# maotian123/loc_lib

Hardware: AMD Instinct MI355X
Metric: scans/sec (64x1800-pt scan vs 10M-pt map) + ICP iter ms (higher is better)
Workload: dtype f64; 1 GPU; BASELINE configs[2]: 256 scans/GPU x 115200 pts (64x1800, cityblock-v1) vs one 10000000-pt map, P2PLANE ICP, reference defaults (alpha=0.1 KD-tree ANN, eps=1e-2, max 20 iters), scans sharded by rank, no collective; includes scan H2D: every step aligns a batch copied host->HBM for it (pinned double buffer, copy stream, overlapped with the previous step); 3 alignment(s) in flight; scans_per_gpu=256, map_points=10000000, pipeline_depth=3, search_mode=tree_faithful_ann, tree_depth=30, tree_bytes=239999992

## Files before the change

### loc_lib_amd/csrc/icp_kernels.hip

```cpp
#include "icp_kernels.hpp"
#include "launch.hpp"
#include "search_walk.hpp"
#include "../../include/locgpu.h"

#include <algorithm>
#include <cstdlib>

namespace locgpu {

template <int KMAX, int D, bool COUNT>
__global__ __launch_bounds__(kBlock) void icp_search_kernel(const uint2* __restrict__ tree, const float4* __restrict__ src,
                                                            const int* __restrict__ counts, const PoseState* __restrict__ st,
                                                            uint32_t* __restrict__ nn, size_t nn_pitch, int max_n, int k, float alpha_eff,
                                                            int skip_nonfinite, unsigned long long* __restrict__ visit_totals, uint32_t* __restrict__ touched,
                                                            const int* __restrict__ active, const int* __restrict__ src_of) {
    __shared__ uint32_t s_far[D][kBlock];
    __shared__ float s_d2[D][kBlock];
    const int scan = active ? active[blockIdx.y] : (int)blockIdx.y;
    if (st[scan].done) return;
    const int tid = threadIdx.x;
    const int i = blockIdx.x * kBlock + tid;
    if (i >= counts[scan]) return;
    const size_t gi = (size_t)scan * max_n + i;
    const float4 p = src[(size_t)(src_of ? src_of[scan] : scan) * max_n + i];
// ... 47 lines not shown
}

template <int K>
__device__ __forceinline__ bool walk_exact_in_wave(const uint2* __restrict__ tree, bool slow, float qx, float qy, float qz, float alpha_eff, uint2* lds,
                                                   uint32_t* __restrict__ nn, size_t nn_pitch, size_t gi, unsigned long long* __restrict__ search_stats) {
    const unsigned long long slow_mask = __ballot(slow);
    if (slow_mask == 0ull || __popcll(slow_mask) > 2) return slow_mask == 0ull;
    if (slow) {
        uint32_t(*s_far)[2] = reinterpret_cast<uint32_t(*)[2]>(lds);
        float(*s_d2)[2] = reinterpret_cast<float(*)[2]>(reinterpret_cast<char*>(lds) + 64 * 2 * sizeof(uint32_t));
        const int col = __popcll(slow_mask & ((1ull << (threadIdx.x & 63)) - 1ull));
        KnnHeap<K> heap;
        uint32_t nvis = 0, lvis = 0, out[K];
        int cnt;
        tree_knn_flat<K, 64, false, 2>(tree, qx, qy, qz, K, alpha_eff, s_far, s_d2, col, heap, nvis, lvis);
        heap_to_sorted<K>(heap, out, cnt);
#pragma unroll
        for (int j = 0; j < K; ++j) nn[(size_t)j * nn_pitch + gi] = out[j];
        if (search_stats) atomicAdd(&search_stats[1], 1ull);
    }
    return true;
}

template <int K, int DF, int LANES = 64, bool STAMP = false, int WIN = 0>
__global__ __launch_bounds__(64) void icp_search_walk_kernel(const uint2* __restrict__ tree, const float4* __restrict__ src,
                                                             const int* __restrict__ counts, const PoseState* __restrict__ st,
                                                             uint32_t* __restrict__ nn, size_t nn_pitch, int max_n, float alpha_eff, int T,
                                                             unsigned int tree_bytes, uint32_t dummy, int skip_nonfinite, uint32_t* __restrict__ redo_list,
                                                             unsigned int* __restrict__ redo_count, uint32_t* __restrict__ deep_list,
                                                             unsigned int* __restrict__ deep_count, unsigned long long* __restrict__ search_stats,
                                                             const int* __restrict__ active, const int* __restrict__ src_of) {
    extern __shared__ uint2 s_dyn[];
    constexpr int ROWB = LANES * 8;
    static_assert(DF * ROWB >= 64 * 2 * 8, "exact stack columns do not fit");
    if ((uint32_t)(size_t)s_dyn != 0u) __builtin_trap();
    const int scan = active ? active[blockIdx.y] : (int)blockIdx.y;
    const int tid = threadIdx.x;
    if (st[scan].done) return;
    const int i = blockIdx.x * LANES + tid;
    if (tid >= LANES || i >= counts[scan]) return;
    const size_t gi = (size_t)scan * max_n + i;
    const float4 p = load_once(&src[(size_t)(src_of ? src_of[scan] : scan) * max_n + i]);
    const bool finite = !skip_nonfinite || (isfinite(p.x) && isfinite(p.y) && isfinite(p.z));
    if (search_stats && finite) atomicAdd(&search_stats[0], 1ull);
    const D3 qs = se3_apply(st[scan].q, st[scan].t, D3{(double)p.x, (double)p.y, (double)p.z});
    const __amdgpu_buffer_rsrc_t rsrc = __builtin_amdgcn_make_buffer_rsrc((void*)tree, 0, (int)tree_bytes, 0x00020000);
    Walk<K> w;
    w.qx = (float)qs.x; w.qy = (float)qs.y; w.qz = (float)qs.z;
    static_assert(WIN <= DF - 2, "the window lies in the rows above the two candidate rows");
    walk_query<K, ROWB, STAMP, WIN>(rsrc, tree, w, finite, alpha_eff, T, dummy, (uint32_t)(size_t)(&s_dyn[tid]), DF);
    if (STAMP && search_stats) {
        atomicAdd(&search_stats[4], (unsigned long long)w.rounds);
        if ((tid & 63) == 0) { atomicAdd(&search_stats[9], (unsigned long long)w.wave_rounds); atomicAdd(&search_stats[12], 1ull); }
        atomicAdd(&search_stats[13], (unsigned long long)w.wave_rounds);
        redo_list[nn_pitch + gi] = w.rounds;
    }
    const bool deep = w.c3n == 1u;
    const bool slow = !deep && w.slow != 0u;
    if (!deep && !slow) {
#pragma unroll
        for (int j = 0; j < K; ++j) __builtin_nontemporal_store(w.id[j], &nn[(size_t)j * nn_pitch + gi]);
    }
    wave_append(deep_list, deep_count, deep, (uint32_t)gi);
    if (LANES == 16) {
        bool pending = slow;
        for (;;) {
            const unsigned long long m = __ballot(pending);
            if (m == 0ull) break;
            const bool mine = pending && __popcll(m & ((1ull << (threadIdx.x & 63)) - 1ull)) < 2;
            (void)walk_exact_in_wave<K>(tree, mine, w.qx, w.qy, w.qz, alpha_eff, s_dyn, nn, nn_pitch, gi, search_stats);
            pending = pending && !mine;
        }
    } else if (!walk_exact_in_wave<K>(tree, slow, w.qx, w.qy, w.qz, alpha_eff, s_dyn, nn, nn_pitch, gi, search_stats)) {
        wave_append(redo_list, redo_count, slow, (uint32_t)gi);
    }
}

template <int K, int D, int LANES = 64>
__global__ __launch_bounds__(64) void icp_search_walk_list_kernel(const uint2* __restrict__ tree, const float4* __restrict__ src,
                                                                  const PoseState* __restrict__ st, uint32_t* __restrict__ nn, size_t nn_pitch, int max_n,
                                                                  float alpha_eff, unsigned int tree_bytes, uint32_t dummy, const uint32_t* __restrict__ list,
                                                                  const unsigned int* __restrict__ n_list, uint32_t* __restrict__ redo_list,
                                                                  unsigned int* __restrict__ redo_count, unsigned long long* __restrict__ search_stats,
                                                                  const int* __restrict__ src_of) {
    extern __shared__ uint2 s_dyn[];
    constexpr int ROWB = LANES * 8;
    static_assert((D + 2) * ROWB >= 64 * 2 * 8, "exact stack columns do not fit");
    if ((uint32_t)(size_t)s_dyn != 0u) __builtin_trap();
    const unsigned int n = *n_list;
    const int tid = threadIdx.x;
    if (blockIdx.x == 0 && tid == 0 && search_stats) atomicAdd(&search_stats[2], (unsigned long long)n);
    if (tid >= LANES) return;
    const __amdgpu_buffer_rsrc_t rsrc = __builtin_amdgcn_make_buffer_rsrc((void*)tree, 0, (int)tree_bytes, 0x00020000);
    const unsigned int per_wave = min((unsigned int)LANES, max(1u, (n + gridDim.x - 1) / gridDim.x));
    for (unsigned int r0 = blockIdx.x * per_wave; r0 < n; r0 += gridDim.x * per_wave) {
        const unsigned int r = r0 + (unsigned int)tid;
        const bool valid = (unsigned int)tid < per_wave && r < n;
// ... 159 lines not shown
            double t = s_slice[0][threadIdx.x];
#pragma unroll
            for (int w = 1; w < kBlock / 32; ++w) t += s_slice[w][threadIdx.x];
            dst[threadIdx.x] = t;
        }
    }
};

__device__ __forceinline__ void R_hat(const double* R, const D3& q, double (&Rh)[3][3]) {
#pragma unroll
    for (int r = 0; r < 3; ++r) {
        Rh[r][0] = R[3 * r + 1] * q.z - R[3 * r + 2] * q.y;
        Rh[r][1] = R[3 * r + 2] * q.x - R[3 * r + 0] * q.z;
        Rh[r][2] = R[3 * r + 0] * q.y - R[3 * r + 1] * q.x;
    }
}


template <int FIT>
__global__ __launch_bounds__(kBlock) __attribute__((amdgpu_waves_per_eu(4, 4))) void icp_plane_accum_kernel(const uint2* __restrict__ tree, const float4* __restrict__ src,
                                                                 const int* __restrict__ counts, const PoseState* __restrict__ st,
                                                                 const uint32_t* __restrict__ nn, size_t nn_pitch, int max_n,
                                                                 double max_plane_distance, double* __restrict__ partials, int kPlanePts,
                                                                 const int* __restrict__ active, const int* __restrict__ src_of) {
    __shared__ double s_row[8][kAccPad];
    __shared__ double s_slice[kBlock / 32][32];
    const int scan = active ? active[blockIdx.y] : (int)blockIdx.y;
    if (st[scan].done) return;
    const int tid = threadIdx.x;
    RowAccum ra;
    ra.init();
#pragma unroll 1
    for (int pp = 0; pp < kPlanePts; ++pp) {
        const int i = (blockIdx.x * kPlanePts + pp) * kBlock + tid;
        double J[1][6] = {{0.0, 0.0, 0.0, 0.0, 0.0, 0.0}};
        double neg_e[1] = {0.0};
        double fitted = 0.0;
        if (i < counts[scan]) {
            const size_t gi = (size_t)scan * max_n + i;
            uint32_t slot[5];
#pragma unroll
            for (int j = 0; j < 5; ++j) slot[j] = __builtin_nontemporal_load(&nn[(size_t)j * nn_pitch + gi]);
            const float4 p = src[(size_t)(src_of ? src_of[scan] : scan) * max_n + i];
            if (slot[4] != kInvalidSlot) {
                D3 nb[5];
#pragma unroll
                for (int j = 0; j < 5; ++j) nb[j] = leaf_point(tree, slot[j]);
                double n4[4];
                if constexpr (FIT == 1) {
                    if (!plane_null_vector_secular(nb, n4)) plane_null_vector(nb, n4);
                } else {
                    plane_null_vector(nb, n4);
                }
                const D3 n3{n4[0], n4[1], n4[2]};
                bool fit = true;
#pragma unroll
                for (int j = 0; j < 5; ++j) {
// ... 1 lines not shown
                    if (err * err > 1e-2) fit = false;
                }
                if (fit) {
                    fitted = 1.0;
                    const D3 q{(double)p.x, (double)p.y, (double)p.z};
                    const D3 qs = se3_apply(st[scan].q, st[scan].t, q);
                    const double dis = dot3(n3, qs) + n4[3];
                    if (!(fabs(dis) > max_plane_distance)) {
                        const double* R = st[scan].R;
                        double nR[3];
#pragma unroll
                        for (int c = 0; c < 3; ++c) nR[c] = -n3.x * R[c] + (-n3.y * R[3 + c] + -n3.z * R[6 + c]);
                        J[0][0] = nR[1] * q.z - nR[2] * q.y;
                        J[0][1] = nR[2] * q.x - nR[0] * q.z;
                        J[0][2] = nR[0] * q.y - nR[1] * q.x;
                        J[0][3] = n3.x; J[0][4] = n3.y; J[0][5] = n3.z;
                        neg_e[0] = -dis;
                    }
                }
            }
        }
        ra.add<1>(s_row, J, neg_e, fitted);
    }
    ra.store(s_slice, partials + ((size_t)scan * gridDim.x + blockIdx.x) * kAccW);
}

__global__ __launch_bounds__(kBlock) void icp_point_accum_kernel(const uint2* __restrict__ tree, const float4* __restrict__ src,
                                                                 const int* __restrict__ counts, const PoseState* __restrict__ st,
                                                                 const uint32_t* __restrict__ nn, size_t nn_pitch, int max_n,
                                                                 double max_nn_distance, double* __restrict__ partials, int pts,
                                                                 const int* __restrict__ active, const int* __restrict__ src_of) {
    const int scan = active ? active[blockIdx.y] : (int)blockIdx.y;
    if (st[scan].done) return;
    double acc[28];
#pragma unroll
    for (int v = 0; v < 28; ++v) acc[v] = 0.0;
#pragma unroll 1
    for (int pp = 0; pp < pts; ++pp) {
    const int i = (blockIdx.x * pts + pp) * kBlock + threadIdx.x;
    if (i < counts[scan]) {
        const size_t gi = (size_t)scan * max_n + i;
        const uint32_t s0 = nn[gi];
        if (s0 != kInvalidSlot) {
            const float4 p = src[(size_t)(src_of ? src_of[scan] : scan) * max_n + i];
            const D3 q{(double)p.x, (double)p.y, (double)p.z};
            const D3 qs = se3_apply(st[scan].q, st[scan].t, q);
            const D3 e3 = leaf_point(tree, s0) - qs;
            const double dis2 = dot3(e3, e3);
            if (!(dis2 > max_nn_distance)) {
                acc[27] += 1.0;
                double Rh[3][3];
                R_hat(st[scan].R, q, Rh);
                double J[3][6];
#pragma unroll
                for (int r = 0; r < 3; ++r)
#pragma unroll
                    for (int c = 0; c < 3; ++c) { J[r][c] = Rh[r][c] / 16; J[r][3 + c] = (r == c) ? -1.0 : 0.0; }
                const double e[3] = {e3.x, e3.y, e3.z};
                add_rows<3>(acc, J, e);
            }
        }
    }
    }
    block_reduce_store<28>(acc, partials + ((size_t)scan * gridDim.x + blockIdx.x) * kAccW);
}

__global__ __launch_bounds__(kBlock) void icp_mapplane_accum_kernel(const double4* __restrict__ planes, const float4* __restrict__ src,
                                                                    const int* __restrict__ counts, const PoseState* __restrict__ st,
                                                                    const uint32_t* __restrict__ nn, int max_n, double max_plane_distance,
                                                                    double* __restrict__ partials, int pts, const int* __restrict__ active,
                                                                    const int* __restrict__ src_of) {
    const int scan = active ? active[blockIdx.y] : (int)blockIdx.y;
    if (st[scan].done) return;
    double acc[28];
#pragma unroll
    for (int v = 0; v < 28; ++v) acc[v] = 0.0;
    const int n = counts[scan];
    const size_t region = (size_t)(src_of ? src_of[scan] : scan) * max_n;
#pragma unroll 1
    for (int pp = 0; pp < pts; ++pp) {
        const int i = (blockIdx.x * pts + pp) * kBlock + threadIdx.x;
        if (i < n) {
            const uint32_t s0 = __builtin_nontemporal_load(&nn[(size_t)scan * max_n + i]);
            const float4 p = src[region + i];
            if (s0 != kInvalidSlot) {
                const double4 n4 = planes[s0 >> 1];
                if (n4.x == n4.x) {
                    acc[27] += 1.0;
                    const D3 n3{n4.x, n4.y, n4.z};
                    const D3 q{(double)p.x, (double)p.y, (double)p.z};
                    const D3 qs = se3_apply(st[scan].q, st[scan].t, q);
                    const double dis = dot3(n3, qs) + n4.w;
                    if (!(fabs(dis) > max_plane_distance)) {
                        const double* R = st[scan].R;
                        double nR[3];
#pragma unroll
                        for (int c = 0; c < 3; ++c) nR[c] = -n3.x * R[c] + (-n3.y * R[3 + c] + -n3.z * R[6 + c]);
                        double J[1][6];
                        J[0][0] = nR[1] * q.z - nR[2] * q.y;
                        J[0][1] = nR[2] * q.x - nR[0] * q.z;
                        J[0][2] = nR[0] * q.y - nR[1] * q.x;
                        J[0][3] = n3.x; J[0][4] = n3.y; J[0][5] = n3.z;
                        const double e[1] = {dis};
                        add_rows<1>(acc, J, e);
                    }
                }
            }
        }
    }
    block_reduce_store<28>(acc, partials + ((size_t)scan * gridDim.x + blockIdx.x) * kAccW);
}

__global__ __launch_bounds__(kBlock) __attribute__((amdgpu_waves_per_eu(5, 5))) void icp_line_accum_kernel(const uint2* __restrict__ tree, const float4* __restrict__ src,
                                                                const int* __restrict__ counts, const PoseState* __restrict__ st,
                                                                const uint32_t* __restrict__ nn, size_t nn_pitch, int max_n,
                                                                double max_line_distance, double* __restrict__ partials, int pts,
                                                                const int* __restrict__ active, const int* __restrict__ src_of) {
    __shared__ double s_row[8][kAccPad];
    __shared__ double s_slice[kBlock / 32][32];
    const int scan = active ? active[blockIdx.y] : (int)blockIdx.y;
    if (st[scan].done) return;
    RowAccum ra;
    ra.init();
#pragma unroll 1
    for (int pp = 0; pp < pts; ++pp) {
    const int i = (blockIdx.x * pts + pp) * kBlock + threadIdx.x;
    double J[3][6], neg_e[3] = {0.0, 0.0, 0.0};
    double fitted = 0.0;
#pragma unroll
    for (int r = 0; r < 3; ++r)
#pragma unroll
        for (int c = 0; c < 6; ++c) J[r][c] = 0.0;
    if (i < counts[scan]) {
        const size_t gi = (size_t)scan * max_n + i;
        uint32_t slot[5];
#pragma unroll
        for (int j = 0; j < 5; ++j) slot[j] = nn[(size_t)j * nn_pitch + gi];
        const float4 p = src[(size_t)(src_of ? src_of[scan] : scan) * max_n + i];
        if (slot[4] != kInvalidSlot) {
            const D3 q{(double)p.x, (double)p.y, (double)p.z};
            const D3 qs = se3_apply(st[scan].q, st[scan].t, q);
            D3 nb[5];
#pragma unroll
            for (int j = 0; j < 5; ++j) nb[j] = leaf_point(tree, slot[j]);
            D3 sum{0.0, 0.0, 0.0};
#pragma unroll
            for (int j = 0; j < 5; ++j) sum = sum + nb[j];
            const D3 p0{sum.x / 5.0, sum.y / 5.0, sum.z / 5.0};
            D3 dl[5];
// ... 23 lines not shown
                            s += hd[r][2] * R[6 + c];
                            hR[r][c] = s;
                        }
#pragma unroll
                    for (int r = 0; r < 3; ++r)
#pragma unroll
                        for (int c = 0; c < 3; ++c) {
                            double s = hR[r][0] * hq[0][c];
                            s += hR[r][1] * hq[1][c];
                            s += hR[r][2] * hq[2][c];
                            A[r][c] = s;
                        }
#pragma unroll
                    for (int r = 0; r < 3; ++r)
#pragma unroll
                        for (int c = 0; c < 3; ++c) { J[r][c] = -A[r][c]; J[r][3 + c] = hd[r][c]; }
                    neg_e[0] = -e3.x; neg_e[1] = -e3.y; neg_e[2] = -e3.z;
                }
            }
        }
    }
    ra.add<3>(s_row, J, neg_e, fitted);
    }
    ra.store(s_slice, partials + ((size_t)scan * gridDim.x + blockIdx.x) * kAccW);
}

__device__ __forceinline__ double reduce_partials(const double* __restrict__ rows, int blocks_per_scan, bool mine, double (*s_sum)[kAccW]) {
    const int col = threadIdx.x & (kAccW - 1), chunk = threadIdx.x / kAccW;
    constexpr int kChunks = kBlock / kAccW;
    double s = 0.0;
    if (mine && col < 28) {
        constexpr int kFlight = 32;
        for (int b = chunk; b < blocks_per_scan; b += kChunks * kFlight) {
            double v[kFlight];
#pragma unroll
            for (int u = 0; u < kFlight; ++u) {
                const int idx = b + u * kChunks;
                v[u] = idx < blocks_per_scan ? rows[(size_t)idx * kAccW + col] : 0.0;
            }
#pragma unroll
            for (int u = 0; u < kFlight; ++u) s += v[u];
        }
    }
    s_sum[chunk][col] = s;
    __syncthreads();
    double t = 0.0;
    if (threadIdx.x < kAccW) {
// ... 108 lines not shown
    if ((threadIdx.x & 63) == 0 && c) atomicAdd(&totals[3], c);
}

__global__ __launch_bounds__(kBlock) void transform_cloud_kernel(const float4* __restrict__ src, size_t n, M12f m, float* __restrict__ dst_xyz) {
    const size_t i = (size_t)blockIdx.x * kBlock + threadIdx.x;
    if (i >= n) return;
    const float4 p = src[i];
    const float* m12 = m.v;
    dst_xyz[3 * i + 0] = ((m12[0] * p.x + m12[1] * p.y) + m12[2] * p.z) + m12[3];
    dst_xyz[3 * i + 1] = ((m12[4] * p.x + m12[5] * p.y) + m12[6] * p.z) + m12[7];
    dst_xyz[3 * i + 2] = ((m12[8] * p.x + m12[9] * p.y) + m12[10] * p.z) + m12[11];
}

__global__ __launch_bounds__(kBlock) void nn_to_index_kernel(const uint2* __restrict__ tree, const uint32_t* __restrict__ nn, size_t nn_pitch, size_t n_queries,
                                                             int k, int32_t* __restrict__ out) {
    const size_t gi = (size_t)blockIdx.x * kBlock + threadIdx.x;
    if (gi >= n_queries) return;
    for (int j = 0; j < k; ++j) {
        const uint32_t slot = nn[(size_t)j * nn_pitch + gi];
        out[gi * k + j] = slot == kInvalidSlot ? -1 : (int32_t)(tree[slot].y & 0x3FFFFFFFu);
    }
}

void launch_nn_to_index(const uint2* tree, const uint32_t* nn, size_t nn_pitch, size_t n_queries, int k, int32_t* out, hipStream_t s) {
    hipLaunchKernelGGL(nn_to_index_kernel, dim3((unsigned)((n_queries + kBlock - 1) / kBlock)), dim3(kBlock), 0, s, tree, nn, nn_pitch, n_queries, k, out);
}

template <int KMAX, int D>
static void launch_search_kd(const SearchArgs& a, hipStream_t s) {
    dim3 grid((a.max_n + kBlock - 1) / kBlock, a.active ? a.n_active : a.n_scans);
    if (a.visit_totals)
        hipLaunchKernelGGL((icp_search_kernel<KMAX, D, true>), grid, dim3(kBlock), 0, s, a.tree, a.src, a.counts, a.st, a.nn, a.nn_pitch, a.max_n,
                           a.k, a.alpha_eff, a.skip_nonfinite, a.visit_totals, a.touched, a.active, a.src_of);
    else
        hipLaunchKernelGGL((icp_search_kernel<KMAX, D, false>), grid, dim3(kBlock), 0, s, a.tree, a.src, a.counts, a.st, a.nn, a.nn_pitch, a.max_n,
                           a.k, a.alpha_eff, a.skip_nonfinite, a.visit_totals, nullptr, a.active, a.src_of);
}

template <int KMAX>
static bool launch_search_k(const SearchArgs& a, hipStream_t s) {
    if (a.depth <= 32) launch_search_kd<KMAX, 32>(a, s);
    else if (a.depth <= 40) launch_search_kd<KMAX, 40>(a, s);
    else if (a.depth <= 64) launch_search_kd<KMAX, 64>(a, s);
    else return false;
    return true;
}
static int fast_stack_depth() {
    static int v = -1;
    if (v < 0) {
        const char* e = getenv("LOCGPU_FAST_STACK");
        v = e ? atoi(e) : 10;
        if (v != 12 && v != 15 && v != 24) v = 10;
    }
    return v;
}

template <auto Kernel>
static bool no_static_lds() {
    hipFuncAttributes attr{};
    return hipFuncGetAttributes(&attr, reinterpret_cast<const void*>(Kernel)) == hipSuccess && attr.sharedSizeBytes == 0;
}
template <int K, int D>
static bool walk_kernels_ok_kd() {
    return no_static_lds<icp_search_walk_kernel<K, 10, 64, false, 8>>() && no_static_lds<icp_search_walk_kernel<K, 12>>() && no_static_lds<icp_search_walk_kernel<K, 15>>() && no_static_lds<icp_search_walk_kernel<K, 24>>() &&
           no_static_lds<icp_search_walk_kernel<K, D + 2, 16>>() && no_static_lds<icp_search_walk_list_kernel<K, D, kDeepLanes>>();
}
bool search_kernels_lds_ok() {
    static const bool ok = walk_kernels_ok_kd<1, 32>() && walk_kernels_ok_kd<1, 40>() && walk_kernels_ok_kd<1, 64>() &&
                           walk_kernels_ok_kd<5, 32>() && walk_kernels_ok_kd<5, 40>() && walk_kernels_ok_kd<5, 64>();
    return ok;
}

template <int K, int D, int DF, int WIN = 0>
static bool launch_walk_kd(const SearchArgs& a, hipStream_t s) {
    static const bool stamp = [] { const char* e = getenv("LOCGPU_STAMP"); return e && atoi(e) != 0; }();
    const uint32_t dummy = (uint32_t)(a.tree_bytes / 8);
    const unsigned int rsrc_bytes = (unsigned int)a.tree_bytes + 16u;
    const int n_launch = a.active ? a.n_active : a.n_scans;
    if (!stamp && (size_t)((a.max_n + 63) / 64) * n_launch <= 2048) {
        dim3 g1((a.max_n + 15) / 16, n_launch);
        hipLaunchKernelGGL((icp_search_walk_kernel<K, D + 2, 16>), g1, dim3(64), (D + 2) * 16 * 8, s, a.tree, a.src, a.counts, a.st, a.nn, a.nn_pitch, a.max_n,
                           a.alpha_eff, 0, rsrc_bytes, dummy, a.skip_nonfinite, a.redo_list, a.redo_count, a.redo_list2, a.redo_count2, a.search_stats, a.active, a.src_of);
        return true;
    }
    static const int t_off = [] { const char* e = getenv("LOCGPU_K1_T_OFFSET"); const int v = e ? atoi(e) : 0; return v > 0 ? v : 13; }();
    const int stored = WIN ? t_off : DF - 2;
    const int Tw = a.depth > stored ? a.depth - stored : 0;
    dim3 g2((a.max_n + 63) / 64, n_launch);
    static const bool lds_knob = getenv("LOCGPU_K1_LDS_BYTES") != nullptr;
    unsigned lds_bytes = DF * 64 * 8;
    if (lds_knob) { const char* e = getenv("LOCGPU_K1_LDS_BYTES"); lds_bytes = (unsigned)std::max(e ? atoi(e) : 0, DF * 64 * 8); }
    if (stamp)
        hipLaunchKernelGGL((icp_search_walk_kernel<K, DF, 64, true, WIN>), g2, dim3(64), DF * 64 * 8, s, a.tree, a.src, a.counts, a.st, a.nn, a.nn_pitch, a.max_n,
                           a.alpha_eff, Tw, rsrc_bytes, dummy, a.skip_nonfinite, a.redo_list, a.redo_count, a.redo_list2, a.redo_count2, a.search_stats, a.active, a.src_of);
    else
        hipLaunchKernelGGL((icp_search_walk_kernel<K, DF, 64, false, WIN>), g2, dim3(64), lds_bytes, s, a.tree, a.src, a.counts, a.st, a.nn, a.nn_pitch, a.max_n,
                           a.alpha_eff, Tw, rsrc_bytes, dummy, a.skip_nonfinite, a.redo_list, a.redo_count, a.redo_list2, a.redo_count2, a.search_stats, a.active, a.src_of);
    hipLaunchKernelGGL((icp_search_walk_list_kernel<K, D, kDeepLanes>), dim3(kDeepWaves), dim3(64), (D + 2) * kDeepLanes * 8, s, a.tree, a.src, a.st, a.nn, a.nn_pitch, a.max_n,
                       a.alpha_eff, rsrc_bytes, dummy, a.redo_list2, a.redo_count2, a.redo_list, a.redo_count, a.search_stats, a.src_of);
    hipLaunchKernelGGL((icp_search_redo_kernel<K, D>), dim3(kRedoWaves), dim3(64), 0, s, a.tree, a.src, a.st, a.nn, a.nn_pitch, a.max_n, a.k,
                       a.alpha_eff, a.redo_list, a.redo_count, a.search_stats, a.src_of);
    return true;
}
template <int K, int D>
static bool launch_walk_d(const SearchArgs& a, hipStream_t s) {
    switch (fast_stack_depth()) {
        default: {
            static const int win = [] { const char* e = getenv("LOCGPU_K1_WIN"); return e ? atoi(e) : 8; }();
            if (win == 6) return launch_walk_kd<K, D, 10, 6>(a, s);
            if (win == 7) return launch_walk_kd<K, D, 10, 7>(a, s);
            return launch_walk_kd<K, D, 10, 8>(a, s);
        }
        case 12: {
            static const int win = [] { const char* e = getenv("LOCGPU_K1_WIN"); return e ? atoi(e) : 0; }();
            if (win == 8) return launch_walk_kd<K, D, 12, 8>(a, s);
            if (win == 9) return launch_walk_kd<K, D, 12, 9>(a, s);
            return launch_walk_kd<K, D, 12>(a, s);
        }
        case 24: return launch_walk_kd<K, D, 24>(a, s);
        case 15: return launch_walk_kd<K, D, 15>(a, s);
// ... 70 lines not shown
    if (depth <= 32) hipLaunchKernelGGL((knn_query_kernel<KMAX, 32>), grid, dim3(kBlock), 0, s, tree, q, nq, k, alpha_eff, out, visits);
    else if (depth <= 40) hipLaunchKernelGGL((knn_query_kernel<KMAX, 40>), grid, dim3(kBlock), 0, s, tree, q, nq, k, alpha_eff, out, visits);
    else if (depth <= 64) hipLaunchKernelGGL((knn_query_kernel<KMAX, 64>), grid, dim3(kBlock), 0, s, tree, q, nq, k, alpha_eff, out, visits);
    else return false;
    return true;
}
bool launch_knn_query(const uint2* tree, int depth, const float* q, size_t nq, int k, float alpha_eff, int32_t* out, uint32_t* visits,
                      hipStream_t s) {
    if (k == 1) return launch_knn_k<1>(tree, depth, q, nq, k, alpha_eff, out, visits, s);
    if (k <= 5) return launch_knn_k<5>(tree, depth, q, nq, k, alpha_eff, out, visits, s);
    if (k <= 8) return launch_knn_k<8>(tree, depth, q, nq, k, alpha_eff, out, visits, s);
    return false;
}

int icp_accum_split(int method, int max_n, int n_scans) {
    const long total_blocks = (long)((max_n + kBlock - 1) / kBlock) * n_scans;
    return total_blocks >= 8192 ? (method == 2 ? 4 : 8) : (total_blocks >= 4096 ? 4 : (total_blocks >= 2048 ? 2 : 1));
}

int launch_icp_accum(int method, const AccumArgs& a, hipStream_t s) {
    const int blocks = (a.max_n + kBlock - 1) / kBlock;
    int pts = icp_accum_split(method, a.max_n, a.n_scans);
    if (a.split_scans > 0) pts = icp_accum_split(method, a.max_n, a.split_scans);
    const dim3 grid((blocks + pts - 1) / pts, a.active ? a.n_active : a.n_scans);
    if (method == 2) {
        if (plane_fit_mode() == 1)
            hipLaunchKernelGGL(icp_plane_accum_kernel<1>, grid, dim3(kBlock), 0, s, a.tree, a.src, a.counts, a.st, a.nn, a.nn_pitch, a.max_n, a.gate, a.partials, pts, a.active, a.src_of);
        else
            hipLaunchKernelGGL(icp_plane_accum_kernel<0>, grid, dim3(kBlock), 0, s, a.tree, a.src, a.counts, a.st, a.nn, a.nn_pitch, a.max_n, a.gate, a.partials, pts, a.active, a.src_of);
    } else if (method == LOCGPU_P2PLANE_MAP)
        hipLaunchKernelGGL(icp_mapplane_accum_kernel, grid, dim3(kBlock), 0, s, reinterpret_cast<const double4*>(a.planes), a.src, a.counts, a.st, a.nn, a.max_n, a.gate, a.partials, pts, a.active, a.src_of);
    else if (method == 1)
        hipLaunchKernelGGL(icp_line_accum_kernel, grid, dim3(kBlock), 0, s, a.tree, a.src, a.counts, a.st, a.nn, a.nn_pitch, a.max_n, a.gate, a.partials, pts, a.active, a.src_of);
    else
        hipLaunchKernelGGL(icp_point_accum_kernel, grid, dim3(kBlock), 0, s, a.tree, a.src, a.counts, a.st, a.nn, a.nn_pitch, a.max_n, a.gate, a.partials, pts, a.active, a.src_of);
    return (int)grid.x;
}

void launch_gn_solve(const double* partials, int blocks_per_scan, PoseState* st, int n_scans, const GnParams& prm, int do_update, double* hb_out,
                     unsigned int* list_counts, hipStream_t s, const int* scans, const GnPost* post) {
    hipLaunchKernelGGL(gn_solve_kernel, dim3(n_scans), dim3(kBlock), 0, s, partials, blocks_per_scan, st, prm, do_update, hb_out, list_counts, scans, post ? *post : GnPost{});
}

void launch_sum_partials(const double* partials, int blocks_per_scan, const PoseState* st_all, int first, int n_local, int n_total, double* acc,
                         hipStream_t s, const unsigned char* owned) {
    hipLaunchKernelGGL(sum_partials_kernel, dim3(n_total), dim3(kBlock), 0, s, partials, blocks_per_scan, st_all, first, n_local, acc, owned);
}

void launch_count_touched(uint32_t* touched, size_t n_words, unsigned long long* totals, hipStream_t s) {
    hipLaunchKernelGGL(count_touched_kernel, dim3(1024), dim3(kBlock), 0, s, touched, n_words, totals);
}

void launch_transform_cloud(const float4* src, size_t n, const M12f& m12, float* dst_xyz, hipStream_t s) {
    hipLaunchKernelGGL(transform_cloud_kernel, dim3((unsigned)((n + kBlock - 1) / kBlock)), dim3(kBlock), 0, s, src, n, m12, dst_xyz);
}

}
```

### loc_lib_amd/csrc/icp_kernels.hpp

```cpp
#pragma once
#include <hip/hip_runtime.h>
#include <stdint.h>

#include "device_math.hpp"

namespace locgpu {

constexpr int kBlock = 256;
constexpr int kAccW = 32;
constexpr uint32_t kInvalidSlot = 0xFFFFFFFFu;
constexpr int kSearchStatSlots = 16 + 2 * 64;

struct GnParams {
    int method;
    int max_iteration;
    int min_effective_pts;
    double eps;
    double max_nn_distance, max_plane_distance, max_line_distance;
    bool operator==(const GnParams& o) const {
        return method == o.method && max_iteration == o.max_iteration && min_effective_pts == o.min_effective_pts && eps == o.eps &&
               max_nn_distance == o.max_nn_distance && max_plane_distance == o.max_plane_distance && max_line_distance == o.max_line_distance;
    }
};

__device__ __forceinline__ float as_f32(uint32_t u) { return __uint_as_float(u); }

__device__ __forceinline__ void wave_append(uint32_t* __restrict__ list, unsigned int* __restrict__ count, bool pred, uint32_t value) {
    const unsigned long long mask = __ballot(pred);
    if (!mask) return;
    const int lane = (int)__lane_id();
    const int leader = __ffsll((long long)mask) - 1;
    unsigned int base = 0;
    if (lane == leader) base = atomicAdd(count, (unsigned int)__popcll(mask));
    base = (unsigned int)__shfl((int)base, leader, 64);
    if (pred) list[base + (unsigned int)__popcll(mask & ((1ull << lane) - 1ull))] = value;
}

template <int KMAX>
struct KnnHeap {
    float d[KMAX + 1];
    uint32_t id[KMAX + 1];
    int n;

    __device__ __forceinline__ float getd(int i) const {
        float r = d[0];
// ... 213 lines not shown
```

### loc_lib_amd/csrc/launch.hpp

```cpp
#pragma once
#include "gn_post.hpp"
#include <hip/hip_runtime.h>
#include <stdint.h>

#include "device_math.hpp"

namespace locgpu {

struct GnParams;

struct SearchArgs {
    const uint2* tree;
    size_t tree_bytes;
    int depth;
    const float4* src;
    const int* counts;
    const PoseState* st;
    uint32_t* nn;
    size_t nn_pitch;
    int max_n, n_scans, k;
    float alpha_eff;
    int skip_nonfinite;
    unsigned long long* visit_totals;
    uint32_t* redo_list;
// ... 4 lines not shown
    const int* active = nullptr;
    int n_active = 0;
    const int* src_of = nullptr;
    uint32_t* touched = nullptr;
};

struct AccumArgs {
    const uint2* tree;
    const float4* src;
    const int* counts;
    const PoseState* st;
    const uint32_t* nn;
    size_t nn_pitch;
    int max_n, n_scans;
    double gate;
    double* partials;
    const int* active = nullptr;
    int n_active = 0;
    const int* src_of = nullptr;
    int split_scans = 0;
    const double* planes = nullptr;
};

bool launch_icp_search(const SearchArgs& a, hipStream_t s);
bool launch_icp_search_redo(const SearchArgs& a, hipStream_t s);
bool launch_icp_search_list(const SearchArgs& a, const uint32_t* list, const unsigned int* n_list, hipStream_t s);
bool launch_knn_query(const uint2* tree, int depth, const float* q, size_t nq, int k, float alpha_eff, int32_t* out, uint32_t* visits,
                      hipStream_t s);
int launch_icp_accum(int method, const AccumArgs& a, hipStream_t s);
void launch_gn_solve(const double* partials, int blocks_per_scan, PoseState* st, int n_scans, const GnParams& prm, int do_update, double* hb_out,
                     unsigned int* list_counts, hipStream_t s, const int* scans = nullptr, const GnPost* post = nullptr);
int icp_accum_split(int method, int max_n, int n_scans);
void launch_sum_partials(const double* partials, int blocks_per_scan, const PoseState* st_all, int first, int n_local, int n_total, double* acc,
                         hipStream_t s, const unsigned char* owned = nullptr);
constexpr int kFitW = 4;
struct FitnessArgs {
    const uint2* tree;
    const float4* src;
    const int* counts;
    const PoseState* st;
    const uint32_t* nn;
    int max_n, n_scans;
    float gate2;
    double* partials;
    double* out;
    unsigned int* list_counts;
// ... 17 lines not shown
```

### loc_lib_amd/csrc/locgpu_api.hip

```cpp
#include <algorithm>
#include <atomic>
#include <chrono>
#include <thread>
#include <cmath>
#include <cstdio>
#include <cstring>
#include <string>
#include <vector>

#include "batch_upload.hpp"
#include "context.hpp"
#include "cloud_filters.hpp"
#include "kdtree_build.hpp"
#include "launch.hpp"

#include <dlfcn.h>
#include <rccl/rccl.h>

using namespace locgpu;

namespace {
struct Rccl {
    ncclResult_t (*GetUniqueId)(ncclUniqueId*) = nullptr;
    ncclResult_t (*CommInitRank)(ncclComm_t*, int, ncclUniqueId, int) = nullptr;
// ... 155 lines not shown
int locgpu_create(int device_id, locgpu_ctx** out) {
    if (!out) return fail(nullptr, LOCGPU_ERR_INVALID, "locgpu_create: out is NULL");
    *out = nullptr;
    int n = 0;
    hipError_t e = hipGetDeviceCount(&n);
    if (e != hipSuccess || n <= 0)
        return fail(nullptr, LOCGPU_ERR_NO_DEVICE, std::string("no HIP device available (there is no CPU fallback): ") + hipGetErrorString(e));
    if (device_id < 0 || device_id >= n) return fail(nullptr, LOCGPU_ERR_INVALID, "locgpu_create: device_id out of range");
    auto* ctx = new locgpu_ctx();
    ctx->device = device_id;
    locgpu_ndt_opts_default(&ctx->ndt_opts);
    bool ok = hip_ok(nullptr, hipSetDevice(device_id), "hipSetDevice");
    for (int i = 0; ok && i < locgpu_ctx::kSlots; ++i) ok = hip_ok(nullptr, hipStreamCreateWithFlags(&ctx->slot_stream[i], hipStreamNonBlocking), "hipStreamCreate");
    ok = ok && hip_ok(nullptr, hipStreamCreateWithFlags(&ctx->copy_stream, hipStreamNonBlocking), "hipStreamCreate");
    ok = ok && hip_ok(nullptr, hipStreamCreateWithFlags(&ctx->comm_stream, hipStreamNonBlocking), "hipStreamCreate");
    if (!ok) {
        for (hipStream_t st : ctx->slot_stream) if (st) (void)hipStreamDestroy(st);
        if (ctx->copy_stream) (void)hipStreamDestroy(ctx->copy_stream);
        if (ctx->comm_stream) (void)hipStreamDestroy(ctx->comm_stream);
        delete ctx;
        return LOCGPU_ERR_NO_DEVICE;
    }
    ctx->stream = ctx->slot_stream[0];
    if (!search_kernels_lds_ok()) {
        locgpu_destroy(ctx);
        return fail(nullptr, LOCGPU_ERR_INVALID, "locgpu_create: a search kernel of this build owns static LDS — its traversal stack would not start at LDS address 0 (search_walk.hpp)");
    }
    *out = ctx;
    return LOCGPU_OK;
}

void locgpu_destroy(locgpu_ctx* ctx) {
    if (!ctx) return;
    (void)hipSetDevice(ctx->device);
    (void)target_join(ctx, false);
    free_target_scratch(ctx);
    for (hipStream_t st : ctx->slot_stream) if (st) (void)hipStreamSynchronize(st);
    if (ctx->comm_stream) (void)hipStreamSynchronize(ctx->comm_stream);
    delete ctx->worker;
    free_batch(ctx->single);
    free_batch(ctx->search);
    free_batch(ctx->planes_ws);
    if (ctx->d_planes) (void)hipFree(ctx->d_planes);
    if (ctx->d_planes_count) (void)hipFree(ctx->d_planes_count);
    upload_free_ctx(ctx);
    if (ctx->comm) { (void)rccl().CommDestroy((ncclComm_t)ctx->comm); ctx->comm = nullptr; }
// ... 1819 lines not shown
```

Before: 12140 scans/s.

## Flatten search walk and accumulate kernels into grid-stride loops over virtual tiles

The walk-search kernel and the ICP accumulate kernels now launch a flat 1-D grid. Each block loops over a virtual (scan, tile) index described by a new VGrid struct, instead of reading blockIdx.x/y directly. The grid size can be capped at a per-CU multiple of the device CU count, queried at context creation, or set through environment knobs. The per-CU constants are zero, so by default the grid still equals the total tile count. The walk kernel also gains an amdgpu_waves_per_eu(8) occupancy hint, which can change register allocation. The change lays groundwork for persistent, machine-sized grids, at the cost of an integer divide per tile and extra __syncthreads in the accumulate loops.

```diff
diff --git a/loc_lib_amd/csrc/icp_kernels.hip b/loc_lib_amd/csrc/icp_kernels.hip
--- a/loc_lib_amd/csrc/icp_kernels.hip
+++ b/loc_lib_amd/csrc/icp_kernels.hip
@@ -93,22 +93,17 @@
     return true;
 }
 
-template <int K, int DF, int LANES = 64, bool STAMP = false, int WIN = 0>
-__global__ __launch_bounds__(64) void icp_search_walk_kernel(const uint2* __restrict__ tree, const float4* __restrict__ src,
-                                                             const int* __restrict__ counts, const PoseState* __restrict__ st,
-                                                             uint32_t* __restrict__ nn, size_t nn_pitch, int max_n, float alpha_eff, int T,
-                                                             unsigned int tree_bytes, uint32_t dummy, int skip_nonfinite, uint32_t* __restrict__ redo_list,
-                                                             unsigned int* __restrict__ redo_count, uint32_t* __restrict__ deep_list,
-                                                             unsigned int* __restrict__ deep_count, unsigned long long* __restrict__ search_stats,
-                                                             const int* __restrict__ active, const int* __restrict__ src_of) {
-    extern __shared__ uint2 s_dyn[];
+template <int K, int DF, int LANES, bool STAMP, int WIN>
+__device__ __forceinline__ void walk_tile(uint2* s_dyn, int scan, int tile, const uint2* __restrict__ tree, const float4* __restrict__ src,
+                                          const int* __restrict__ counts, const PoseState* __restrict__ st, uint32_t* __restrict__ nn, size_t nn_pitch,
+                                          int max_n, float alpha_eff, int T, unsigned int tree_bytes, uint32_t dummy, int skip_nonfinite,
+                                          uint32_t* __restrict__ redo_list, unsigned int* __restrict__ redo_count, uint32_t* __restrict__ deep_list,
+                                          unsigned int* __restrict__ deep_count, unsigned long long* __restrict__ search_stats,
+                                          const int* __restrict__ src_of) {
     constexpr int ROWB = LANES * 8;
-    static_assert(DF * ROWB >= 64 * 2 * 8, "exact stack columns do not fit");
-    if ((uint32_t)(size_t)s_dyn != 0u) __builtin_trap();
-    const int scan = active ? active[blockIdx.y] : (int)blockIdx.y;
     const int tid = threadIdx.x;
     if (st[scan].done) return;
-    const int i = blockIdx.x * LANES + tid;
+    const int i = tile * LANES + tid;
     if (tid >= LANES || i >= counts[scan]) return;
     const size_t gi = (size_t)scan * max_n + i;
     const float4 p = load_once(&src[(size_t)(src_of ? src_of[scan] : scan) * max_n + i]);
@@ -144,6 +139,32 @@
         }
     } else if (!walk_exact_in_wave<K>(tree, slow, w.qx, w.qy, w.qz, alpha_eff, s_dyn, nn, nn_pitch, gi, search_stats)) {
         wave_append(redo_list, redo_count, slow, (uint32_t)gi);
+    }
+}
+
+template <int K, int DF, int LANES = 64, bool STAMP = false, int WIN = 0, bool LOOP = false>
+__global__ __launch_bounds__(64) __attribute__((amdgpu_waves_per_eu(8))) void icp_search_walk_kernel(const uint2* __restrict__ tree, const float4* __restrict__ src,
+                                                             const int* __restrict__ counts, const PoseState* __restrict__ st,
+                                                             uint32_t* __restrict__ nn, size_t nn_pitch, int max_n, float alpha_eff, int T,
+                                                             unsigned int tree_bytes, uint32_t dummy, int skip_nonfinite, uint32_t* __restrict__ redo_list,
+                                                             unsigned int* __restrict__ redo_count, uint32_t* __restrict__ deep_list,
+                                                             unsigned int* __restrict__ deep_count, unsigned long long* __restrict__ search_stats,
+                                                             const int* __restrict__ active, const int* __restrict__ src_of, VGrid vg) {
+    extern __shared__ uint2 s_dyn[];
+    static_assert(DF * LANES * 8 >= 64 * 2 * 8, "exact stack columns do not fit");
+    if ((uint32_t)(size_t)s_dyn != 0u) __builtin_trap();
+    if constexpr (LOOP) {
+#pragma unroll 1
+        for (int v = blockIdx.x; v < vg.total; v += gridDim.x) {
+            const int vy = v / vg.per_scan, vx = v - vy * vg.per_scan;
+            const int scan = active ? active[vy] : vy;
+            walk_tile<K, DF, LANES, STAMP, WIN>(s_dyn, scan, vx, tree, src, counts, st, nn, nn_pitch, max_n, alpha_eff, T, tree_bytes, dummy, skip_nonfinite,
+                                                redo_list, redo_count, deep_list, deep_count, search_stats, src_of);
+        }
+    } else {
+        const int scan = active ? active[blockIdx.y] : (int)blockIdx.y;
+        walk_tile<K, DF, LANES, STAMP, WIN>(s_dyn, scan, (int)blockIdx.x, tree, src, counts, st, nn, nn_pitch, max_n, alpha_eff, T, tree_bytes, dummy, skip_nonfinite,
+                                            redo_list, redo_count, deep_list, deep_count, search_stats, src_of);
     }
 }
 
@@ -349,17 +370,20 @@
                                                                  const int* __restrict__ counts, const PoseState* __restrict__ st,
                                                                  const uint32_t* __restrict__ nn, size_t nn_pitch, int max_n,
                                                                  double max_plane_distance, double* __restrict__ partials, int kPlanePts,
-                                                                 const int* __restrict__ active, const int* __restrict__ src_of) {
+                                                                 const int* __restrict__ active, const int* __restrict__ src_of, VGrid vg) {
     __shared__ double s_row[8][kAccPad];
     __shared__ double s_slice[kBlock / 32][32];
-    const int scan = active ? active[blockIdx.y] : (int)blockIdx.y;
-    if (st[scan].done) return;
     const int tid = threadIdx.x;
+#pragma unroll 1
+    for (int v = blockIdx.x; v < vg.total; v += gridDim.x) {
+    const int vy = v / vg.per_scan, vx = v - vy * vg.per_scan;
+    const int scan = active ? active[vy] : vy;
+    if (st[scan].done) continue;
     RowAccum ra;
     ra.init();
 #pragma unroll 1
     for (int pp = 0; pp < kPlanePts; ++pp) {
-        const int i = (blockIdx.x * kPlanePts + pp) * kBlock + tid;
+        const int i = (vx * kPlanePts + pp) * kBlock + tid;
         double J[1][6] = {{0.0, 0.0, 0.0, 0.0, 0.0, 0.0}};
         double neg_e[1] = {0.0};
         double fitted = 0.0;
@@ -407,22 +431,26 @@
         }
         ra.add<1>(s_row, J, neg_e, fitted);
     }
-    ra.store(s_slice, partials + ((size_t)scan * gridDim.x + blockIdx.x) * kAccW);
+    ra.store(s_slice, partials + ((size_t)scan * vg.per_scan + vx) * kAccW);
+    }
 }
 
 __global__ __launch_bounds__(kBlock) void icp_point_accum_kernel(const uint2* __restrict__ tree, const float4* __restrict__ src,
                                                                  const int* __restrict__ counts, const PoseState* __restrict__ st,
                                                                  const uint32_t* __restrict__ nn, size_t nn_pitch, int max_n,
                                                                  double max_nn_distance, double* __restrict__ partials, int pts,
-                                                                 const int* __restrict__ active, const int* __restrict__ src_of) {
-    const int scan = active ? active[blockIdx.y] : (int)blockIdx.y;
-    if (st[scan].done) return;
+                                                                 const int* __restrict__ active, const int* __restrict__ src_of, VGrid vg) {
+#pragma unroll 1
+    for (int vb = blockIdx.x; vb < vg.total; vb += gridDim.x) {
+    const int vy = vb / vg.per_scan, vx = vb - vy * vg.per_scan;
+    const int scan = active ? active[vy] : vy;
+    if (st[scan].done) continue;
     double acc[28];
 #pragma unroll
     for (int v = 0; v < 28; ++v) acc[v] = 0.0;
 #pragma unroll 1
     for (int pp = 0; pp < pts; ++pp) {
-    const int i = (blockIdx.x * pts + pp) * kBlock + threadIdx.x;
+    const int i = (vx * pts + pp) * kBlock + threadIdx.x;
     if (i < counts[scan]) {
         const size_t gi = (size_t)scan * max_n + i;
         const uint32_t s0 = nn[gi];
@@ -447,16 +475,21 @@
         }
     }
     }
-    block_reduce_store<28>(acc, partials + ((size_t)scan * gridDim.x + blockIdx.x) * kAccW);
+    block_reduce_store<28>(acc, partials + ((size_t)scan * vg.per_scan + vx) * kAccW);
+    __syncthreads();
+    }
 }
 
 __global__ __launch_bounds__(kBlock) void icp_mapplane_accum_kernel(const double4* __restrict__ planes, const float4* __restrict__ src,
                                                                     const int* __restrict__ counts, const PoseState* __restrict__ st,
                                                                     const uint32_t* __restrict__ nn, int max_n, double max_plane_distance,
                                                                     double* __restrict__ partials, int pts, const int* __restrict__ active,
-                                                                    const int* __restrict__ src_of) {
-    const int scan = active ? active[blockIdx.y] : (int)blockIdx.y;
-    if (st[scan].done) return;
+                                                                    const int* __restrict__ src_of, VGrid vg) {
+#pragma unroll 1
+    for (int vb = blockIdx.x; vb < vg.total; vb += gridDim.x) {
+    const int vy = vb / vg.per_scan, vx = vb - vy * vg.per_scan;
+    const int scan = active ? active[vy] : vy;
+    if (st[scan].done) continue;
     double acc[28];
 #pragma unroll
     for (int v = 0; v < 28; ++v) acc[v] = 0.0;
@@ -464,7 +497,7 @@
     const size_t region = (size_t)(src_of ? src_of[scan] : scan) * max_n;
 #pragma unroll 1
     for (int pp = 0; pp < pts; ++pp) {
-        const int i = (blockIdx.x * pts + pp) * kBlock + threadIdx.x;
+        const int i = (vx * pts + pp) * kBlock + threadIdx.x;
         if (i < n) {
             const uint32_t s0 = __builtin_nontemporal_load(&nn[(size_t)scan * max_n + i]);
             const float4 p = src[region + i];
@@ -493,23 +526,28 @@
             }
         }
     }
-    block_reduce_store<28>(acc, partials + ((size_t)scan * gridDim.x + blockIdx.x) * kAccW);
+    block_reduce_store<28>(acc, partials + ((size_t)scan * vg.per_scan + vx) * kAccW);
+    __syncthreads();
+    }
 }
 
 __global__ __launch_bounds__(kBlock) __attribute__((amdgpu_waves_per_eu(5, 5))) void icp_line_accum_kernel(const uint2* __restrict__ tree, const float4* __restrict__ src,
                                                                 const int* __restrict__ counts, const PoseState* __restrict__ st,
                                                                 const uint32_t* __restrict__ nn, size_t nn_pitch, int max_n,
                                                                 double max_line_distance, double* __restrict__ partials, int pts,
-                                                                const int* __restrict__ active, const int* __restrict__ src_of) {
+                                                                const int* __restrict__ active, const int* __restrict__ src_of, VGrid vg) {
     __shared__ double s_row[8][kAccPad];
     __shared__ double s_slice[kBlock / 32][32];
-    const int scan = active ? active[blockIdx.y] : (int)blockIdx.y;
-    if (st[scan].done) return;
+#pragma unroll 1
+    for (int vb = blockIdx.x; vb < vg.total; vb += gridDim.x) {
+    const int vy = vb / vg.per_scan, vx = vb - vy * vg.per_scan;
+    const int scan = active ? active[vy] : vy;
+    if (st[scan].done) continue;
     RowAccum ra;
     ra.init();
 #pragma unroll 1
     for (int pp = 0; pp < pts; ++pp) {
-    const int i = (blockIdx.x * pts + pp) * kBlock + threadIdx.x;
+    const int i = (vx * pts + pp) * kBlock + threadIdx.x;
     double J[3][6], neg_e[3] = {0.0, 0.0, 0.0};
     double fitted = 0.0;
 #pragma unroll
@@ -579,7 +617,8 @@
     }
     ra.add<3>(s_row, J, neg_e, fitted);
     }
-    ra.store(s_slice, partials + ((size_t)scan * gridDim.x + blockIdx.x) * kAccW);
+    ra.store(s_slice, partials + ((size_t)scan * vg.per_scan + vx) * kAccW);
+    }
 }
 
 __device__ __forceinline__ double reduce_partials(const double* __restrict__ rows, int blocks_per_scan, bool mine, double (*s_sum)[kAccW]) {
@@ -734,6 +773,21 @@
     }
 }
 
+
+static int g_machine_cus = 0;
+void launch_set_machine(int compute_units) { g_machine_cus = compute_units; }
+constexpr int kWalkWavesPerCu = 0, kFitBlocksPerCu = 0;
+static int env_grid(const char* name, bool& present_at_first) {
+    if (!present_at_first) return 0;
+    const char* e = getenv(name);
+    const int v = e ? atoi(e) : 0;
+    return v > 0 ? v : 0;
+}
+static unsigned machine_grid(int total, int per_cu, const char* knob, bool& knob_present) {
+    int g = env_grid(knob, knob_present);
+    if (g <= 0) g = (g_machine_cus > 0 && per_cu > 0) ? g_machine_cus * per_cu : total;
+    return (unsigned)std::max(1, std::min(g, total));
+}
 void launch_nn_to_index(const uint2* tree, const uint32_t* nn, size_t nn_pitch, size_t n_queries, int k, int32_t* out, hipStream_t s) {
     hipLaunchKernelGGL(nn_to_index_kernel, dim3((unsigned)((n_queries + kBlock - 1) / kBlock)), dim3(kBlock), 0, s, tree, nn, nn_pitch, n_queries, k, out);
 }
@@ -772,9 +826,14 @@
     hipFuncAttributes attr{};
     return hipFuncGetAttributes(&attr, reinterpret_cast<const void*>(Kernel)) == hipSuccess && attr.sharedSizeBytes == 0;
 }
+template <int K, int DF, int WIN>
+static bool walk_loop_ok() {
+    return no_static_lds<icp_search_walk_kernel<K, DF, 64, false, WIN, true>>() && no_static_lds<icp_search_walk_kernel<K, DF, 64, true, WIN, true>>();
+}
 template <int K, int D>
 static bool walk_kernels_ok_kd() {
-    return no_static_lds<icp_search_walk_kernel<K, 10, 64, false, 8>>() && no_static_lds<icp_search_walk_kernel<K, 12>>() && no_static_lds<icp_search_walk_kernel<K, 15>>() && no_static_lds<icp_search_walk_kernel<K, 24>>() &&
+    return walk_loop_ok<K, 10, 6>() && walk_loop_ok<K, 10, 7>() && walk_loop_ok<K, 10, 8>() && walk_loop_ok<K, 12, 0>() && walk_loop_ok<K, 12, 8>() &&
+           walk_loop_ok<K, 12, 9>() && walk_loop_ok<K, 15, 0>() && walk_loop_ok<K, 24, 0>() &&
            no_static_lds<icp_search_walk_kernel<K, D + 2, 16>>() && no_static_lds<icp_search_walk_list_kernel<K, D, kDeepLanes>>();
 }
 bool search_kernels_lds_ok() {
@@ -792,22 +851,24 @@
     if (!stamp && (size_t)((a.max_n + 63) / 64) * n_launch <= 2048) {
         dim3 g1((a.max_n + 15) / 16, n_launch);
         hipLaunchKernelGGL((icp_search_walk_kernel<K, D + 2, 16>), g1, dim3(64), (D + 2) * 16 * 8, s, a.tree, a.src, a.counts, a.st, a.nn, a.nn_pitch, a.max_n,
-                           a.alpha_eff, 0, rsrc_bytes, dummy, a.skip_nonfinite, a.redo_list, a.redo_count, a.redo_list2, a.redo_count2, a.search_stats, a.active, a.src_of);
+                           a.alpha_eff, 0, rsrc_bytes, dummy, a.skip_nonfinite, a.redo_list, a.redo_count, a.redo_list2, a.redo_count2, a.search_stats, a.active, a.src_of, VGrid{});
         return true;
     }
     static const int t_off = [] { const char* e = getenv("LOCGPU_K1_T_OFFSET"); const int v = e ? atoi(e) : 0; return v > 0 ? v : 13; }();
     const int stored = WIN ? t_off : DF - 2;
     const int Tw = a.depth > stored ? a.depth - stored : 0;
-    dim3 g2((a.max_n + 63) / 64, n_launch);
+    const VGrid vg{(a.max_n + 63) / 64, (a.max_n + 63) / 64 * n_launch};
+    static bool grid_knob = getenv("LOCGPU_K1_GRID") != nullptr;
+    const dim3 g2(machine_grid(vg.total, kWalkWavesPerCu, "LOCGPU_K1_GRID", grid_knob));
     static const bool lds_knob = getenv("LOCGPU_K1_LDS_BYTES") != nullptr;
     unsigned lds_bytes = DF * 64 * 8;
     if (lds_knob) { const char* e = getenv("LOCGPU_K1_LDS_BYTES"); lds_bytes = (unsigned)std::max(e ? atoi(e) : 0, DF * 64 * 8); }
     if (stamp)
-        hipLaunchKernelGGL((icp_search_walk_kernel<K, DF, 64, true, WIN>), g2, dim3(64), DF * 64 * 8, s, a.tree, a.src, a.counts, a.st, a.nn, a.nn_pitch, a.max_n,
-                           a.alpha_eff, Tw, rsrc_bytes, dummy, a.skip_nonfinite, a.redo_list, a.redo_count, a.redo_list2, a.redo_count2, a.search_stats, a.active, a.src_of);
+        hipLaunchKernelGGL((icp_search_walk_kernel<K, DF, 64, true, WIN, true>), g2, dim3(64), DF * 64 * 8, s, a.tree, a.src, a.counts, a.st, a.nn, a.nn_pitch, a.max_n,
+                           a.alpha_eff, Tw, rsrc_bytes, dummy, a.skip_nonfinite, a.redo_list, a.redo_count, a.redo_list2, a.redo_count2, a.search_stats, a.active, a.src_of, vg);
     else
-        hipLaunchKernelGGL((icp_search_walk_kernel<K, DF, 64, false, WIN>), g2, dim3(64), lds_bytes, s, a.tree, a.src, a.counts, a.st, a.nn, a.nn_pitch, a.max_n,
-                           a.alpha_eff, Tw, rsrc_bytes, dummy, a.skip_nonfinite, a.redo_list, a.redo_count, a.redo_list2, a.redo_count2, a.search_stats, a.active, a.src_of);
+        hipLaunchKernelGGL((icp_search_walk_kernel<K, DF, 64, false, WIN, true>), g2, dim3(64), lds_bytes, s, a.tree, a.src, a.counts, a.st, a.nn, a.nn_pitch, a.max_n,
+                           a.alpha_eff, Tw, rsrc_bytes, dummy, a.skip_nonfinite, a.redo_list, a.redo_count, a.redo_list2, a.redo_count2, a.search_stats, a.active, a.src_of, vg);
     hipLaunchKernelGGL((icp_search_walk_list_kernel<K, D, kDeepLanes>), dim3(kDeepWaves), dim3(64), (D + 2) * kDeepLanes * 8, s, a.tree, a.src, a.st, a.nn, a.nn_pitch, a.max_n,
                        a.alpha_eff, rsrc_bytes, dummy, a.redo_list2, a.redo_count2, a.redo_list, a.redo_count, a.search_stats, a.src_of);
     hipLaunchKernelGGL((icp_search_redo_kernel<K, D>), dim3(kRedoWaves), dim3(64), 0, s, a.tree, a.src, a.st, a.nn, a.nn_pitch, a.max_n, a.k,
@@ -924,19 +985,22 @@
     const int blocks = (a.max_n + kBlock - 1) / kBlock;
     int pts = icp_accum_split(method, a.max_n, a.n_scans);
     if (a.split_scans > 0) pts = icp_accum_split(method, a.max_n, a.split_scans);
-    const dim3 grid((blocks + pts - 1) / pts, a.active ? a.n_active : a.n_scans);
+    const int per_scan = (blocks + pts - 1) / pts;
+    const VGrid vg{per_scan, per_scan * (a.active ? a.n_active : a.n_scans)};
+    static bool grid_knob = getenv("LOCGPU_K2_GRID") != nullptr;
+    const dim3 grid(machine_grid(vg.total, kFitBlocksPerCu, "LOCGPU_K2_GRID", grid_knob));
     if (method == 2) {
         if (plane_fit_mode() == 1)
-            hipLaunchKernelGGL(icp_plane_accum_kernel<1>, grid, dim3(kBlock), 0, s, a.tree, a.src, a.counts, a.st, a.nn, a.nn_pitch, a.max_n, a.gate, a.partials, pts, a.active, a.src_of);
+            hipLaunchKernelGGL(icp_plane_accum_kernel<1>, grid, dim3(kBlock), 0, s, a.tree, a.src, a.counts, a.st, a.nn, a.nn_pitch, a.max_n, a.gate, a.partials, pts, a.active, a.src_of, vg);
         else
-            hipLaunchKernelGGL(icp_plane_accum_kernel<0>, grid, dim3(kBlock), 0, s, a.tree, a.src, a.counts, a.st, a.nn, a.nn_pitch, a.max_n, a.gate, a.partials, pts, a.active, a.src_of);
+            hipLaunchKernelGGL(icp_plane_accum_kernel<0>, grid, dim3(kBlock), 0, s, a.tree, a.src, a.counts, a.st, a.nn, a.nn_pitch, a.max_n, a.gate, a.partials, pts, a.active, a.src_of, vg);
     } else if (method == LOCGPU_P2PLANE_MAP)
-        hipLaunchKernelGGL(icp_mapplane_accum_kernel, grid, dim3(kBlock), 0, s, reinterpret_cast<const double4*>(a.planes), a.src, a.counts, a.st, a.nn, a.max_n, a.gate, a.partials, pts, a.active, a.src_of);
+        hipLaunchKernelGGL(icp_mapplane_accum_kernel, grid, dim3(kBlock), 0, s, reinterpret_cast<const double4*>(a.planes), a.src, a.counts, a.st, a.nn, a.max_n, a.gate, a.partials, pts, a.active, a.src_of, vg);
     else if (method == 1)
-        hipLaunchKernelGGL(icp_line_accum_kernel, grid, dim3(kBlock), 0, s, a.tree, a.src, a.counts, a.st, a.nn, a.nn_pitch, a.max_n, a.gate, a.partials, pts, a.active, a.src_of);
+        hipLaunchKernelGGL(icp_line_accum_kernel, grid, dim3(kBlock), 0, s, a.tree, a.src, a.counts, a.st, a.nn, a.nn_pitch, a.max_n, a.gate, a.partials, pts, a.active, a.src_of, vg);
     else
-        hipLaunchKernelGGL(icp_point_accum_kernel, grid, dim3(kBlock), 0, s, a.tree, a.src, a.counts, a.st, a.nn, a.nn_pitch, a.max_n, a.gate, a.partials, pts, a.active, a.src_of);
-    return (int)grid.x;
+        hipLaunchKernelGGL(icp_point_accum_kernel, grid, dim3(kBlock), 0, s, a.tree, a.src, a.counts, a.st, a.nn, a.nn_pitch, a.max_n, a.gate, a.partials, pts, a.active, a.src_of, vg);
+    return per_scan;
 }
 
 void launch_gn_solve(const double* partials, int blocks_per_scan, PoseState* st, int n_scans, const GnParams& prm, int do_update, double* hb_out,
diff --git a/loc_lib_amd/csrc/icp_kernels.hpp b/loc_lib_amd/csrc/icp_kernels.hpp
--- a/loc_lib_amd/csrc/icp_kernels.hpp
+++ b/loc_lib_amd/csrc/icp_kernels.hpp
@@ -21,6 +21,11 @@
         return method == o.method && max_iteration == o.max_iteration && min_effective_pts == o.min_effective_pts && eps == o.eps &&
                max_nn_distance == o.max_nn_distance && max_plane_distance == o.max_plane_distance && max_line_distance == o.max_line_distance;
     }
+};
+
+struct VGrid {
+    int per_scan;
+    int total;
 };
 
 __device__ __forceinline__ float as_f32(uint32_t u) { return __uint_as_float(u); }
diff --git a/loc_lib_amd/csrc/launch.hpp b/loc_lib_amd/csrc/launch.hpp
--- a/loc_lib_amd/csrc/launch.hpp
+++ b/loc_lib_amd/csrc/launch.hpp
@@ -50,6 +50,7 @@
     const double* planes = nullptr;
 };
 
+void launch_set_machine(int compute_units);
 bool launch_icp_search(const SearchArgs& a, hipStream_t s);
 bool launch_icp_search_redo(const SearchArgs& a, hipStream_t s);
 bool launch_icp_search_list(const SearchArgs& a, const uint32_t* list, const unsigned int* n_list, hipStream_t s);
diff --git a/loc_lib_amd/csrc/locgpu_api.hip b/loc_lib_amd/csrc/locgpu_api.hip
--- a/loc_lib_amd/csrc/locgpu_api.hip
+++ b/loc_lib_amd/csrc/locgpu_api.hip
@@ -201,6 +201,10 @@
         return LOCGPU_ERR_NO_DEVICE;
     }
     ctx->stream = ctx->slot_stream[0];
+    {
+        int cus = 0;
+        if (hipDeviceGetAttribute(&cus, hipDeviceAttributeMultiprocessorCount, device_id) == hipSuccess && cus > 0) launch_set_machine(cus);
+    }
     if (!search_kernels_lds_ok()) {
         locgpu_destroy(ctx);
         return fail(nullptr, LOCGPU_ERR_INVALID, "locgpu_create: a search kernel of this build owns static LDS — its traversal stack would not start at LDS address 0 (search_walk.hpp)");
```

After: 11800 scans/s. -2.8%, worse.
